# xyyandhtl/IsaacgymLoco

Hardware: AMD Instinct MI355X
Metric: env-steps/sec (whole node) (higher is better)
Workload: dtype f32; 1 GPU; aliengo: HIMOnPolicyRunner loop, 9 whole PPO iteration(s) timed, each = 100 x (policy inference + LeggedRobot.step + storage) + GAE + HIMPPO.update (5 epochs x 4 minibatches), 4096 envs/GPU; task=aliengo, envs_per_gpu=4096, mode=train, parallelism=dp1, mixed_robots=False, full=False

## Files before the change

### include/lsim.h

```cpp
#ifndef LSIM_H
#define LSIM_H

#include <stddef.h>
#include <stdint.h>

#ifdef __cplusplus
extern "C" {
#endif

#define LSIM_ABI_VERSION 7

#define LSIM_NUM_DOF 12
#define LSIM_NUM_BODIES 17
#define LSIM_NUM_LEGS 4
#define LSIM_NUM_ACTIONS 12
#define LSIM_ONE_STEP_OBS 45
#define LSIM_OBS_HISTORY 6
#define LSIM_NUM_OBS 270
#define LSIM_MAX_HEIGHT_PTS_X 32
#define LSIM_MAX_HEIGHT_PTS_Y 32
#define LSIM_NUM_HEIGHT_PTS 187
#define LSIM_NUM_PRIV_OBS 238
#define LSIM_NUM_AMP_OBS 30
#define LSIM_NUM_BASE_HEIGHT_PTS 63
// ... 473 lines not shown


int lsim_adaptive_lr(const float* kl_mean_dev, float desired_kl, float lr_min, float lr_max, float factor, float* lr_dev, void* stream);

int lsim_sinkhorn_workspace(long batch, int K, size_t* bytes);
int lsim_sinkhorn(const float* scores, int64_t lds, int64_t batch, int K, float eps, int iters, float* out,
                  void* workspace, size_t workspace_bytes, void* stream);

int lsim_estimator_loss_workspace(int64_t batch, int latent, int K, size_t* bytes);
int lsim_estimator_loss(const float* enc_out, int64_t ld_enc, const float* tgt_out, int64_t ld_tgt, const float* proto, const float* vel,
                        int64_t ld_vel, int64_t batch, int latent, int K, float temperature, float sinkhorn_eps, int sinkhorn_iters,
                        float* losses3, float* grad_enc, float* grad_tgt, float* grad_proto, void* workspace, size_t workspace_bytes,
                        void* stream);

int lsim_adam_clip_step_workspace(int count, size_t* bytes);
int lsim_adam_clip_step(int count, const int64_t* numel, float* const* params, float* const* grads, float* const* exp_avg,
                        float* const* exp_avg_sq, float* const* steps, const float* lr_dev, float lr_host, float beta1, float beta2,
                        float eps, float max_grad_norm, float* grad_norm_out, void* workspace, size_t workspace_bytes, void* stream);

int lsim_adam_clip_step_ex(int count, const int64_t* numel, float* const* params, float* const* grads, float* const* exp_avg,
                           float* const* exp_avg_sq, float* const* steps, const float* weight_decay, int clip_count,
                           const float* lr_dev, float lr_host, float beta1, float beta2, float eps, float max_grad_norm,
                           float* grad_norm_out, void* workspace, size_t workspace_bytes, void* stream);

int lsim_actor_input(const float* obs, int64_t ld_obs, int num_one_step_obs, const float* enc_out, int64_t ld_enc, int latent,
                     int64_t batch, float* out, void* stream);

#define LSIM_EVAL_BY_ROBOT 1u
#define LSIM_EVAL_BY_TYPE 2u
#define LSIM_EVAL_BY_LEVEL 4u
#define LSIM_EVAL_MAX_GROUPS 4096
#define LSIM_EVAL_MAX_TRACE_ENVS 64
#define LSIM_EVAL_SAT_PERMILLE 980
enum lsim_eval_word {
    LSIM_EVAL_W_SAMPLES = 0,
    LSIM_EVAL_W_LIN_ERR,
    LSIM_EVAL_W_LIN_ERR_SQ,
    LSIM_EVAL_W_YAW_ERR,
    LSIM_EVAL_W_YAW_ERR_SQ,
    LSIM_EVAL_W_POWER,
    LSIM_EVAL_W_TORQUE_SQ,
    LSIM_EVAL_W_ACTION_RATE,
    LSIM_EVAL_W_FEET_CONTACT,
    LSIM_EVAL_W_TORQUE_SAT,
    LSIM_EVAL_W_PEAK_TORQUE_RATIO,
    LSIM_EVAL_W_EPISODES,
// ... 516 lines not shown
```

### isaacgymloco_amd/abi.py

```python
import ctypes
import os
import re

_HERE = os.path.dirname(os.path.abspath(__file__))
REPO_ROOT = os.path.dirname(_HERE)
HEADER_PATH = os.path.join(REPO_ROOT, "include", "lsim.h")

_CTYPES = {
    "float": ctypes.c_float, "double": ctypes.c_double,
    "int32_t": ctypes.c_int32, "uint32_t": ctypes.c_uint32,
    "int64_t": ctypes.c_int64, "uint64_t": ctypes.c_uint64,
    "int16_t": ctypes.c_int16, "uint8_t": ctypes.c_uint8, "int": ctypes.c_int,
}


def _strip_comments(text):
    text = re.sub(r"/\*.*?\*/", "", text, flags=re.S)
    return re.sub(r"//[^\n]*", "", text)


def _parse(text, overrides=None):
    text = _strip_comments(text)
    defines = {}
    for m in re.finditer(r"^\s*#define\s+(\w+)\s+(.+?)\s*$", text, flags=re.M):
# ... 48 lines not shown
                decl = decl.strip()
                dm = re.match(r"(\w+)((?:\[[^\]]+\])*)$", decl)
                name, dims = dm.group(1), re.findall(r"\[([^\]]+)\]", dm.group(2))
                ct = base
                for d in reversed(dims):
                    ct = ct * int(eval(d, {}, defines))
                fields.append((name, ct))
        structs[m.group(3)] = type(m.group(3), (ctypes.Structure,), {"_fields_": fields})
    return defines, enums, structs


with open(HEADER_PATH) as _f:
    DEFINES, ENUMS, STRUCTS = _parse(_f.read())

LsimConfig = STRUCTS["lsim_config"]
LsimRobotModel = STRUCTS["lsim_robot_model"]
LsimBody = STRUCTS["lsim_body"]
LsimCollisionPoint = STRUCTS["lsim_collision_point"]
LsimRolloutStorage = STRUCTS["lsim_rollout_storage"]
LsimMlpLayer = STRUCTS["lsim_mlp_layer"]
LsimHimPolicy = STRUCTS["lsim_him_policy"]
LsimPolicyExtra = STRUCTS["lsim_policy_extra"]
LsimWgradPending = STRUCTS["lsim_wgrad_pending"]
LsimAmpDisc = STRUCTS["lsim_amp_disc"]
LsimEval = STRUCTS["lsim_eval"]
LsimEvalColumns = STRUCTS["lsim_eval_columns"]
LsimRaycast = STRUCTS["lsim_raycast_t"]
LsimRaycastBodies = STRUCTS["lsim_raycast_bodies_t"]
LsimRaycastRobot = STRUCTS["lsim_raycast_robot"]
LsimRaycastPrim = STRUCTS["lsim_raycast_prim"]
LsimSensorModel = STRUCTS["lsim_sensor_model_t"]
LsimSensorMountJitter = STRUCTS["lsim_sensor_mount_jitter_t"]
LsimSensorInstrument = STRUCTS["lsim_sensor_instrument_t"]
LsimSensorStereo = STRUCTS["lsim_sensor_stereo_t"]
LsimSensorShade = STRUCTS["lsim_sensor_shade_t"]
LsimElevationMap = STRUCTS["lsim_elevation_map_t"]
LsimOdometry = STRUCTS["lsim_odometry_t"]
LsimMapRows = STRUCTS["lsim_map_rows_t"]
LsimElevationMapFused = STRUCTS["lsim_elevation_map_fused_t"]
LsimMapRowsFused = STRUCTS["lsim_map_rows_fused_t"]
LsimElevationMapCleanup = STRUCTS["lsim_elevation_map_cleanup_t"]
LsimFootScan = STRUCTS["lsim_foot_scan_t"]
LsimDepthEncoder = STRUCTS["lsim_depth_encoder_t"]
LsimDepthEncoderBwd = STRUCTS["lsim_depth_encoder_bwd_t"]
LsimFramesLog = STRUCTS["lsim_frames_log_t"]
LsimLatentRowsGrad = STRUCTS["lsim_latent_rows_grad_t"]
# ... 89 lines not shown
```

### isaacgymloco_amd/csrc/ls_learn.h

```cpp
#pragma once
#include <hip/hip_runtime.h>

typedef float ls_v4f __attribute__((ext_vector_type(4)));

#define LS_WGRAD_WAVES_PER_BLOCK 4

template <int NT, int KT>
__global__ __launch_bounds__(64 * LS_WGRAD_WAVES_PER_BLOCK) void lsim_k_linear_wgrad(const float* __restrict__ x, long ldx, const float* __restrict__ g, long ldg,
                                                                                    long batch, int k_in, int n_out, long rows_per_wave,
                                                                                    float* __restrict__ part_dw, float* __restrict__ part_db) {
    const int lane = threadIdx.x & 63, wave = blockIdx.x * LS_WGRAD_WAVES_PER_BLOCK + (threadIdx.x >> 6);
    const int sub = lane >> 4, col = lane & 15;
    const long b0 = (long)wave * rows_per_wave;
    if (b0 >= batch) return;
    long b1 = b0 + rows_per_wave;
    if (b1 > batch) b1 = batch;
    ls_v4f acc[NT][KT];
    float dbacc[NT];
#pragma unroll
    for (int nt = 0; nt < NT; ++nt) {
        dbacc[nt] = 0.0f;
#pragma unroll
        for (int kt = 0; kt < KT; ++kt) acc[nt][kt] = (ls_v4f){0.0f, 0.0f, 0.0f, 0.0f};
    }
// ... 1428 lines not shown
    *bytes = (size_t)((batch + 255) / 256) * (4 + num_actions) * sizeof(float);
    return LSIM_OK;
}
extern "C" int lsim_ppo_loss_std(const float* mu, const float* std, const float* value, const float* actions, const float* old_logp, const float* advantages,
                                 const float* returns, const float* target_values, const float* old_mu, const float* old_sigma, int64_t batch, int num_actions,
                                 float clip_param, float value_loss_coef, float entropy_coef, int use_clipped_value_loss,
                                 float* out5, float* grad_mu, float* grad_std, float* grad_value, void* workspace, size_t workspace_bytes, void* stream) {
    size_t need;
    if (lsim_ppo_loss_std_workspace(batch, num_actions, &need) != LSIM_OK) return LSIM_E_INVALID;
    if (!mu || !std || !value || !actions || !old_logp || !advantages || !returns || !old_mu || !old_sigma || !out5 || !grad_mu || !grad_std ||
        !grad_value || !workspace || workspace_bytes < need || (use_clipped_value_loss && !target_values)) return LSIM_E_INVALID;
    LsPpoLossArgs a;
    a.mu = mu; a.sigma = std; a.value = value; a.actions = actions; a.old_logp = old_logp; a.adv = advantages; a.returns = returns;
    a.target_values = target_values; a.old_mu = old_mu; a.old_sigma = old_sigma; a.g_mu = grad_mu; a.g_sigma = nullptr; a.g_value = grad_value;
    a.partial = (float*)workspace; a.batch = batch; a.A = num_actions; a.clip = clip_param; a.value_coef = value_loss_coef;
    a.entropy_coef = entropy_coef; a.clipped_value = use_clipped_value_loss; a.std_mode = 1;
    const int blocks = (int)((batch + 255) / 256);
    hipLaunchKernelGGL(lsim_k_ppo_loss, dim3(blocks), dim3(256), 0, (hipStream_t)stream, a);
    hipLaunchKernelGGL(lsim_k_ppo_loss_finish_std, dim3(1), dim3(256), 0, (hipStream_t)stream, (const float*)workspace, blocks, (long)batch, num_actions,
                       value_loss_coef, entropy_coef, out5, grad_std);
    return hipGetLastError() == hipSuccess ? LSIM_OK : LSIM_E_HIP;
}

__global__ void lsim_k_adaptive_lr(const float* __restrict__ kl_mean, float desired_kl, float lr_min, float lr_max, float factor, float* __restrict__ lr) {
    const float k = *kl_mean;
    float l = *lr;
    if (k > 2.0f * desired_kl) l = fmaxf(lr_min, l / factor);
    else if (k < 0.5f * desired_kl && k > 0.0f) l = fminf(lr_max, l * factor);
    *lr = l;
}

extern "C" int lsim_adaptive_lr(const float* kl_mean_dev, float desired_kl, float lr_min, float lr_max, float factor, float* lr_dev, void* stream) {
    if (!kl_mean_dev || !lr_dev || desired_kl <= 0.0f || factor <= 1.0f || lr_min <= 0.0f || lr_max < lr_min) return LSIM_E_INVALID;
    hipLaunchKernelGGL(lsim_k_adaptive_lr, dim3(1), dim3(1), 0, (hipStream_t)stream, kl_mean_dev, desired_kl, lr_min, lr_max, factor, lr_dev);
    return hipGetLastError() == hipSuccess ? LSIM_OK : LSIM_E_HIP;
}

#define LS_ADAM_MAX_TENSORS 48
#define LS_ADAM_SLICES 32
struct LsAdamTable {
    float* p[LS_ADAM_MAX_TENSORS];
    float* g[LS_ADAM_MAX_TENSORS];
    float* m[LS_ADAM_MAX_TENSORS];
    float* v[LS_ADAM_MAX_TENSORS];
    float* step[LS_ADAM_MAX_TENSORS];
    int n[LS_ADAM_MAX_TENSORS];
    float wd[LS_ADAM_MAX_TENSORS];
    int count;
    int clip_count;
};

__global__ __launch_bounds__(256) void lsim_k_adam_sumsq(LsAdamTable t, float* __restrict__ part ) {
    __shared__ float red[256];
    const int ti = blockIdx.y, n = t.n[ti];
    const float* __restrict__ g = t.g[ti];
    float s = 0.0f;
    for (int i = blockIdx.x * 256 + threadIdx.x; i < n; i += LS_ADAM_SLICES * 256) { const float x = g[i]; s = fmaf(x, x, s); }
    red[threadIdx.x] = s;
    __syncthreads();
    for (int st = 128; st > 0; st >>= 1) {
        if ((int)threadIdx.x < st) red[threadIdx.x] += red[threadIdx.x + st];
        __syncthreads();
    }
    if (threadIdx.x == 0) {
        part[ti * LS_ADAM_SLICES + blockIdx.x] = red[0];
        if (blockIdx.x == 0) *t.step[ti] += 1.0f;
    }
}

__global__ __launch_bounds__(256) void lsim_k_adam_apply(LsAdamTable t, const float* __restrict__ part, float max_norm, float* __restrict__ scal,
                                                         const float* __restrict__ lr_dev, float lr_host, float b1, float b2, float eps) {
    __shared__ float tot[LS_ADAM_MAX_TENSORS];
    __shared__ float coef_s;
    if ((int)threadIdx.x < t.count) {
        float s = 0.0f;
        for (int k = 0; k < LS_ADAM_SLICES; ++k) s += part[threadIdx.x * LS_ADAM_SLICES + k];
        tot[threadIdx.x] = s;
    }
    __syncthreads();
    if (threadIdx.x == 0) {
        float s = 0.0f;
        for (int k = 0; k < t.clip_count; ++k) s += tot[k];
        const float norm = sqrtf(s);
        coef_s = max_norm > 0.0f ? fminf(max_norm / (norm + 1e-6f), 1.0f) : 1.0f;
        if (blockIdx.x == 0 && blockIdx.y == 0) { scal[0] = coef_s; scal[1] = norm; scal[2] = *t.step[0]; }
    }
    __syncthreads();
    const int ti = blockIdx.y, n = t.n[ti];
    float* __restrict__ p = t.p[ti];
    float* __restrict__ g = t.g[ti];
    float* __restrict__ m = t.m[ti];
    float* __restrict__ v = t.v[ti];
    const float coef = ti < t.clip_count ? coef_s : 1.0f, step = *t.step[ti], lr = lr_dev ? *lr_dev : lr_host, wd = t.wd[ti];
    const float bc1 = 1.0f - powf(b1, step), bc2s = sqrtf(1.0f - powf(b2, step));
    const float step_size = lr / bc1;
    for (int i = blockIdx.x * 256 + threadIdx.x; i < n; i += LS_ADAM_SLICES * 256) {
        const float gc = g[i] * coef;
        const float gi = wd != 0.0f ? gc + wd * p[i] : gc;
        const float mi = m[i] + (gi - m[i]) * (1.0f - b1);
        const float vi = b2 * v[i] + (1.0f - b2) * gi * gi;
        g[i] = gc; m[i] = mi; v[i] = vi;
        p[i] -= step_size * mi / (sqrtf(vi) / bc2s + eps);
    }
}

extern "C" int lsim_adam_clip_step_workspace(int count, size_t* bytes) {
    if (!bytes || count <= 0 || count > LS_ADAM_MAX_TENSORS) return LSIM_E_INVALID;
    *bytes = ((size_t)count * LS_ADAM_SLICES + 4) * sizeof(float);
    return LSIM_OK;
}

extern "C" int lsim_adam_clip_step_ex(int count, const int64_t* numel, float* const* params, float* const* grads, float* const* exp_avg,
                                      float* const* exp_avg_sq, float* const* steps, const float* weight_decay, int clip_count,
                                      const float* lr_dev, float lr_host, float beta1, float beta2, float eps, float max_grad_norm,
                                      float* grad_norm_out, void* workspace, size_t workspace_bytes, void* stream);
extern "C" int lsim_adam_clip_step(int count, const int64_t* numel, float* const* params, float* const* grads, float* const* exp_avg,
                                   float* const* exp_avg_sq, float* const* steps, const float* lr_dev, float lr_host, float beta1, float beta2,
                                   float eps, float max_grad_norm, float* grad_norm_out, void* workspace, size_t workspace_bytes, void* stream) {
    return lsim_adam_clip_step_ex(count, numel, params, grads, exp_avg, exp_avg_sq, steps, nullptr, count, lr_dev, lr_host, beta1, beta2, eps,
                                  max_grad_norm, grad_norm_out, workspace, workspace_bytes, stream);
}

extern "C" int lsim_adam_clip_step_ex(int count, const int64_t* numel, float* const* params, float* const* grads, float* const* exp_avg,
                                      float* const* exp_avg_sq, float* const* steps, const float* weight_decay, int clip_count,
                                      const float* lr_dev, float lr_host, float beta1, float beta2, float eps, float max_grad_norm,
                                      float* grad_norm_out, void* workspace, size_t workspace_bytes, void* stream) {
    size_t need;
    int rc = lsim_adam_clip_step_workspace(count, &need);
    if (rc != LSIM_OK) return rc;
    if (!numel || !params || !grads || !exp_avg || !exp_avg_sq || !steps || !workspace || workspace_bytes < need || beta1 < 0.0f || beta1 >= 1.0f ||
        beta2 < 0.0f || beta2 >= 1.0f || eps <= 0.0f || clip_count < 0 || clip_count > count)
        return LSIM_E_INVALID;
    LsAdamTable t;
    t.count = count;
    t.clip_count = clip_count;
    for (int i = 0; i < count; ++i) {
        if (!params[i] || !grads[i] || !exp_avg[i] || !exp_avg_sq[i] || !steps[i] || numel[i] <= 0 || numel[i] > 0x7fffffffLL) return LSIM_E_INVALID;
        t.p[i] = params[i]; t.g[i] = grads[i]; t.m[i] = exp_avg[i]; t.v[i] = exp_avg_sq[i]; t.step[i] = steps[i]; t.n[i] = (int)numel[i];
        t.wd[i] = weight_decay ? weight_decay[i] : 0.0f;
        if (t.wd[i] < 0.0f) return LSIM_E_INVALID;
    }
    for (int i = count; i < LS_ADAM_MAX_TENSORS; ++i) { t.p[i] = t.g[i] = t.m[i] = t.v[i] = t.step[i] = nullptr; t.n[i] = 0; t.wd[i] = 0.0f; }
    float* part = (float*)workspace;
    float* scal = part + (size_t)count * LS_ADAM_SLICES;
    hipStream_t s = (hipStream_t)stream;
    hipLaunchKernelGGL(lsim_k_adam_sumsq, dim3(LS_ADAM_SLICES, count), dim3(256), 0, s, t, part);
    hipLaunchKernelGGL(lsim_k_adam_apply, dim3(LS_ADAM_SLICES, count), dim3(256), 0, s, t, (const float*)part, max_grad_norm, scal, lr_dev, lr_host, beta1,
                       beta2, eps);
    if (grad_norm_out && hipMemcpyAsync(grad_norm_out, scal + 1, sizeof(float), hipMemcpyDeviceToDevice, s) != hipSuccess) return LSIM_E_HIP;
    return hipGetLastError() == hipSuccess ? LSIM_OK : LSIM_E_HIP;
}

__global__ __launch_bounds__(256) void lsim_k_actor_input(const float* __restrict__ obs, long ld_obs, int n_one, const float* __restrict__ enc, long ld_enc,
                                                          int n_lat, long batch, float* __restrict__ out) {
    const int W = n_one + 3 + n_lat;
    const long idx = (long)blockIdx.x * 256 + threadIdx.x;
    if (idx >= batch * W) return;
    const long row = idx / W;
    const int c = (int)(idx - row * W);
    float v;
    if (c < n_one) v = obs[row * ld_obs + c];
    else if (c < n_one + 3) v = enc[row * ld_enc + (c - n_one)];
    else {
        const float* z = enc + row * ld_enc + 3;
        float ss = 0.0f;
        for (int k = 0; k < n_lat; ++k) ss = fmaf(z[k], z[k], ss);
        v = z[c - n_one - 3] / fmaxf(sqrtf(ss), 1e-12f);
    }
    out[idx] = v;
}

__global__ __launch_bounds__(256) void lsim_k_actor_input64(const float* __restrict__ obs, long ld_obs, int n_one, const float* __restrict__ enc, long ld_enc,
// ... 27 lines not shown
```

### isaacgymloco_amd/learn/fused_linear.py

```python
import ctypes
import os
import weakref

import torch
import torch.nn as nn
import torch.nn.functional as F

_MIN_BATCH = 4096
_workspaces = {}
_plans = {}
_adam_tables = {}


def _workspace(kind, device, nbytes, floor=0):
    key = (kind, device, torch.cuda.current_stream(device).cuda_stream)
    ws = _workspaces.get(key)
    if ws is None or ws.numel() < nbytes:
        ws = torch.empty(max(int(nbytes), int(floor)), dtype=torch.uint8, device=device)
        _workspaces[key] = ws
    return ws


class GradArena:

# ... 373 lines not shown
    _EstimatorLossFn.last_grads = None
    return total, parts


def backward_losses(*losses):
    tensors, grads, rest = [], [], []
    direct = os.environ.get("LSIM_DIRECT_LOSS_BACKWARD", "1") != "0"
    for l in losses:
        d = getattr(l, "_lsim_direct", None) if direct else None
        if d is None or not all(t.requires_grad for t in d[0]):
            rest.append(l)
        else:
            tensors += list(d[0]); grads += list(d[1])
    if tensors:
        torch.autograd.backward(tensors, grads)
    for l in rest:
        l.backward()


def estimator_loss_supported(latent, K):
    return latent <= 32 and K <= 64


def adam_clip_step_hip(optimizer, max_grad_norm, clip_params=None):
    from .. import lib
    groups = optimizer.param_groups
    g0 = groups[0]
    for grp in groups:
        if grp.get("amsgrad") or grp.get("maximize") or grp.get("differentiable") or grp.get("weight_decay", 0) < 0:
            return False
        same_lr = grp["lr"] is g0["lr"] or (not torch.is_tensor(grp["lr"]) and not torch.is_tensor(g0["lr"]) and grp["lr"] == g0["lr"])
        if grp["betas"] != g0["betas"] or grp["eps"] != g0["eps"] or not same_lr:
            return False
    clip_ids = None if clip_params is None else {id(p) for p in clip_params}
    entries = [(p, float(grp.get("weight_decay", 0))) for grp in groups for p in grp["params"] if p.grad is not None]
    if not entries or len(entries) > 48:
        return False
    if clip_ids is not None:
        entries = [e for e in entries if id(e[0]) in clip_ids] + [e for e in entries if id(e[0]) not in clip_ids]
    n_clip = len(entries) if clip_ids is None else sum(1 for e in entries if id(e[0]) in clip_ids)
    n = len(entries)
    L = lib.load()
    dev = entries[0][0].device
    states = [optimizer.state.get(p) for p, _ in entries]
    for (p, _), st in zip(entries, states):
        if (not st or not p.is_cuda or p.dtype != torch.float32 or not p.is_contiguous() or not p.grad.is_contiguous()
                or not torch.is_tensor(st.get("step")) or not st["step"].is_cuda or st["step"].dtype != torch.float32):
            return False
    key = (n_clip, tuple(p.data_ptr() for p, _ in entries), tuple(p.grad.data_ptr() for p, _ in entries),
           tuple(st["exp_avg"].data_ptr() for st in states), tuple(st["exp_avg_sq"].data_ptr() for st in states),
           tuple(st["step"].data_ptr() for st in states), tuple(w for _, w in entries))
    cached = _adam_tables.get(id(optimizer))
    if cached is not None and cached[0] == key and cached[2]() is optimizer:
        tables = cached[1]
    else:
        tabs = ([], [], [], [], [])
        for (p, _), st in zip(entries, states):
            for tab, t in zip(tabs, (p, p.grad, st["exp_avg"], st["exp_avg_sq"], st["step"])):
                tab.append(t.data_ptr())
        need = ctypes.c_size_t()
        lib.check(L.lsim_adam_clip_step_workspace(n, ctypes.byref(need)), what="lsim_adam_clip_step_workspace")
        arr = lambda v: (ctypes.c_void_p * n)(*v)
        tables = (arr(tabs[0]), arr(tabs[1]), arr(tabs[2]), arr(tabs[3]), arr(tabs[4]), (ctypes.c_int64 * n)(*[p.numel() for p, _ in entries]),
                  (ctypes.c_float * n)(*[w for _, w in entries]), need.value)
        oid = id(optimizer)
        _adam_tables[oid] = (key, tables, weakref.ref(optimizer, lambda _r, oid=oid: _adam_tables.pop(oid, None)))
    ws = _workspace(("adam", id(optimizer)), dev, tables[7])
    lr = g0["lr"]
    lr_dev = lr.data_ptr() if torch.is_tensor(lr) and lr.is_cuda else None
    lr_host = 0.0 if lr_dev is not None else float(lr)
    b1, b2 = g0["betas"]
    lib.check(L.lsim_adam_clip_step_ex(n, tables[5], tables[0], tables[1], tables[2], tables[3], tables[4], tables[6], n_clip, lr_dev, lr_host,
                                       float(b1), float(b2), float(g0["eps"]), float(max_grad_norm), None, ws.data_ptr(), ws.numel(),
                                       torch.cuda.current_stream(dev).cuda_stream), what="lsim_adam_clip_step_ex")
    return True
```

### isaacgymloco_amd/learn/him_ppo.py

```python
import os
import time

import torch
import torch.nn as nn

from . import fused_linear as FL
from .storage import HIMRolloutStorage


_two_stream_memo = {}


def _loaded_tunableop_solutions(device):
    tun = torch.cuda.tunable
    a = torch.zeros(8, 8, device=device)
    torch.mm(a, a)
    table = {}
    for rec in tun.get_results():
        if len(rec) >= 3 and str(rec[0]).startswith("Gemm"):
            table[str(rec[1]).split("_ld_")[0]] = str(rec[2])
    return table


def tunableop_status(device, table_path=None):
# ... 171 lines not shown
        self.collectives += 1
        self.dist.all_reduce(v, op=self.dist.ReduceOp.SUM)
        v = v.to(torch.float32)
        return v[0], v[1], v[2]

    def sum_triple_vec(self, a, b, c):
        if not self.enabled:
            return a, b, c
        v = torch.cat((a.reshape(-1), b.reshape(-1), c.reshape(1))).to(torch.float64)
        self.collectives += 1
        self.dist.all_reduce(v, op=self.dist.ReduceOp.SUM)
        n = a.numel()
        return v[:n].view_as(a), v[n:2 * n].view_as(b), v[2 * n]

    def broadcast_module(self, module):
        if not self.enabled:
            return
        for t in list(module.parameters()) + list(module.buffers()):
            self.dist.broadcast(t.data, src=0)


class _Minibatch:
    __slots__ = ("obs", "next_critic_obs", "old_mu", "old_sigma", "loss", "mu", "sigma", "kl_mean", "surrogate_loss", "value_loss", "early_est", "aux",
                 "est", "swap", "est_params", "ppo_params", "kl", "dist", "bucket")

    def step_joint(self, alg, ac, more_params=()):
        alg._mb_backward(ac, self, more_params)
        alg._mb_reduce(self)
        alg._mb_optim(ac, self)


class HIMPPO:
    def __init__(self, actor_critic, num_learning_epochs=1, num_mini_batches=1, clip_param=0.2, gamma=0.998, lam=0.95,
                 value_loss_coef=1.0, entropy_coef=0.0, learning_rate=1e-3, max_grad_norm=1.0, use_clipped_value_loss=True,
                 schedule="fixed", desired_kl=0.01, device="cpu", dist_ctx=None):
        self.device = device
        self.desired_kl, self.schedule, self.learning_rate = desired_kl, schedule, learning_rate
        self.actor_critic = actor_critic.to(device)
        self.storage = None
        self.optimizer = torch.optim.Adam(self.actor_critic.parameters(), lr=learning_rate)
        self.transition = HIMRolloutStorage.Transition()
        self.clip_param, self.num_learning_epochs, self.num_mini_batches = clip_param, num_learning_epochs, num_mini_batches
        self.value_loss_coef, self.entropy_coef, self.gamma, self.lam = value_loss_coef, entropy_coef, gamma, lam
        self.max_grad_norm, self.use_clipped_value_loss = max_grad_norm, use_clipped_value_loss
        self.dist_ctx = dist_ctx
        self._lr_t = None
        if dist_ctx is not None and dist_ctx.enabled:
# ... 171 lines not shown
        est_ids = {id(p) for p in est_params}
        ppo_params = [p for p in ac.parameters() if p.grad is not None and id(p) not in est_ids]
        more = [p for p in more_params if p.grad is not None]
        mb.est, mb.swap, mb.est_params, mb.ppo_params, mb.kl, mb.bucket = est.detach(), swap.detach(), est_params, ppo_params, extra, None
        mb.dist = (mb.mu, mb.sigma, mb.old_mu, mb.old_sigma) if self._lr_t is None else (None,) * 4
        if ctx is not None:
            slot = self._stats_slot()
            in_place = slot is not None and extra is not None and extra.data_ptr() == slot[3:4].data_ptr()
            mb.bucket = ctx.prepare_bucket(est_live + ppo_params + more, extra=None if in_place else extra, key="all",
                                           n_extra=5 if (extra is not None and extra.is_cuda) else None, extra_at=3)
        elif self._grad_arena() is not None:
            self._arena.bucket("all", est_live + ppo_params + more, 0).adopt()

    def _mb_reduce(self, mb):
        if mb.bucket is None:
            return
        ctx = self.dist_ctx
        got = ctx.finish_bucket(ctx.start_reduce(mb.bucket))
        if mb.kl is not None:
            mb.kl = got[3:4] if got.numel() == 5 else got

    def _mb_optim(self, ac, mb):
        est_mod = ac.estimator
        if self._adaptive:
            self._adapt_lr(*mb.dist, mb.kl.reshape(()), already_global=True)
        if self._lr_t is None:
            est_mod.learning_rate = self.learning_rate
            for g in est_mod.optimizer.param_groups:
                g["lr"] = self.learning_rate
        stepped = False
        if est_mod.fused_step:
            stepped = FL.adam_clip_step_hip(est_mod.optimizer, est_mod.max_grad_norm)
        if not stepped:
            nn.utils.clip_grad_norm_(mb.est_params, est_mod.max_grad_norm)
            est_mod.optimizer.step()
        for p in mb.est_params:
            p.grad = None
        self._clip_and_step(self.optimizer, mb.ppo_params, self.max_grad_norm)

    def _mb_step_single_rank(self, ac, mb, bucket_params, clip_params):
        if self._adaptive:
            self._adapt_lr(mb.mu, mb.sigma, mb.old_mu, mb.old_sigma, mb.kl_mean)
        mb.est, mb.swap = ac.estimator.update(mb.obs, mb.next_critic_obs, lr=None if self._lr_t is not None else self.learning_rate)
        self._extra_losses(mb)
        self.optimizer.zero_grad()
        FL.grad_cycle()
        with FL.deferred_wgrad_reduce():
            FL.backward_losses(mb.loss)
        if FL._arena is not None:
            FL._arena.bucket("ppo", [p for p in bucket_params if p.grad is not None]).adopt()
        self._clip_and_step(self.optimizer, clip_params, self.max_grad_norm)

    _std_direct = True
    _two_stream_forward = True

    def _mb_forward(self, ac, batch, two_streams):
        (obs, critic_obs, actions, next_critic_obs, target_values, advantages, returns, old_logp, old_mu, old_sigma) = batch
        if two_streams:
            cur = torch.cuda.current_stream(obs.device)
            side = self._side_stream(obs.device)
            side.wait_stream(cur)
# ... 24 lines not shown
    _n_stats = 4

    def _sample_stream(self):
        for batch in self.storage.mini_batch_generator(self.num_mini_batches, self.num_learning_epochs):
            yield batch, None

    def _extra_losses(self, mb):
        return ()

    def _after_step(self, ac, mb):
        """behind the optimiser steps of a minibatch"""

    def _stats_row(self, mb):
        return mb.value_loss.detach(), mb.surrogate_loss.detach(), mb.est, mb.swap

    def _result(self, means, mb):
        return means[0], means[1], float(mb.est), float(mb.swap)

    def update(self):
        ac = self.actor_critic
        t_enqueue = time.perf_counter()
        self._grad_arena()
        sums = torch.zeros(self._n_stats, device=self.device)
        dist_on = self.dist_ctx is not None and self.dist_ctx.enabled
        for batch, aux in self._sample_stream():
            obs = batch[0]
            two_streams = (self._two_stream_forward and obs.is_cuda and self._lr_t is not None
                           and self._two_streams(ac.critic, obs.shape[0], dist_on and self.dist_ctx.world > 1))
            mb = self._mb_forward(ac, batch, two_streams)
            mb.aux = aux
            if dist_on or two_streams:
                mb.step_joint(self, ac, self._extra_losses(mb))
            else:
                self._mb_step_single_rank(ac, mb, [p for g in self.optimizer.param_groups for p in g["params"]], ac.parameters())
            self._after_step(ac, mb)
            sums += torch.stack(self._stats_row(mb))
        n = self.num_learning_epochs * self.num_mini_batches
        self.update_enqueue_s = time.perf_counter() - t_enqueue
        if self._lr_t is not None:
            self.learning_rate = float(self._lr_t)
        means = (sums / n).tolist()
        self.storage.clear()
        return self._result(means, mb)
```

### isaacgymloco_amd/learn/hybrid.py

```python
import torch
import torch.nn as nn

from .amp import AMPDiscriminator, AMPLoader, Normalizer, ReplayBuffer, default_motion_files
from .him_ppo import HIMPPO
from .modules import HIMActorCritic
from .runner import HIMOnPolicyRunner
from .storage import HIMRolloutStorage


class HybridPPO(HIMPPO):
    def __init__(self, actor_critic, discriminator, amp_data, amp_normalizer, amp_replay_buffer_size=100000, min_std=None,
                 device="cpu", dist_ctx=None, **kw):
        super().__init__(actor_critic, device=device, dist_ctx=dist_ctx, **kw)
        self.min_std = min_std
        self.discriminator = discriminator.to(device)
        self.amp_transition = HIMRolloutStorage.Transition()
        self.amp_storage = ReplayBuffer(discriminator.input_dim // 2, amp_replay_buffer_size, device)
        self.amp_data, self.amp_normalizer = amp_data, amp_normalizer
        self.optimizer = torch.optim.Adam([
            {"params": self.actor_critic.parameters(), "name": "actor_critic"},
            {"params": self.discriminator.trunk.parameters(), "weight_decay": 10e-4, "name": "amp_trunk"},
            {"params": self.discriminator.amp_linear.parameters(), "weight_decay": 10e-2, "name": "amp_head"}], lr=self.learning_rate)
        if dist_ctx is not None and dist_ctx.enabled:
            dist_ctx.broadcast_module(self.discriminator)
            if amp_normalizer is not None:
                amp_normalizer.moment_sync = lambda a, b, c: tuple(t.to(torch.float64) for t in dist_ctx.sum_triple_vec(a, b, c))

    def act(self, obs, critic_obs, amp_obs):
        self.amp_transition.observations = amp_obs
        return super().act(obs, critic_obs)

    def process_env_step(self, rewards, dones, infos, amp_obs, next_critic_obs):
        self.amp_storage.insert(self.amp_transition.observations, amp_obs)
        self.amp_transition.clear()
        super().process_env_step(rewards, dones, infos, next_critic_obs)

    _std_direct = False
    _two_stream_forward = False
    _n_stats = 6

    def _sample_stream(self):
        n_updates, rows = self.num_learning_epochs * self.num_mini_batches, self.storage.num_envs * self.storage.num_transitions_per_env // self.num_mini_batches
        for sample, policy_pair, expert_pair in zip(self.storage.mini_batch_generator(self.num_mini_batches, self.num_learning_epochs),
                                                    self.amp_storage.feed_forward_generator(n_updates, rows),
                                                    self.amp_data.feed_forward_generator(n_updates, rows)):
            yield sample, (policy_pair, expert_pair)

    def _extra_losses(self, mb):
        disc = self.discriminator
        (pol_s, pol_ns), (exp_s_raw, exp_ns_raw) = mb.aux
        expert_in, policy_in, expert_raw, exp_s, pol_s = disc.pair_inputs(exp_s_raw, exp_ns_raw, pol_s, pol_ns, self.amp_normalizer)
        amp_loss, policy_d_mean, expert_d_mean = disc.lsgan_loss(expert_in, policy_in)
        grad_pen = disc.compute_grad_pen(exp_s_raw, exp_ns_raw, lambda_=10, pair=expert_raw)
        mb.loss = mb.loss + amp_loss + grad_pen
        mb.aux = (pol_s, exp_s, amp_loss.detach(), grad_pen.detach(), policy_d_mean, expert_d_mean)
        return disc.parameters()

    def _after_step(self, ac, mb):
        if self.min_std is not None:
            ac.std.data = ac.std.data.clamp(min=self.min_std)
        if self.amp_normalizer is not None:
# ... 91 lines not shown
```

Before: 4.945 million env-steps/s.

## Fuse adaptive LR, two Adam clip steps and stat accumulation into one tail

Adds a combined update-tail entry point that runs the estimator and PPO Adam clip-steps as two kernels covering both optimizers together. The first kernel also applies the adaptive learning-rate rule and accumulates the per-minibatch loss statistics. The HIM PPO minibatch optimizer path calls it when possible, which removes several small kernel launches and torch.stack/add ops per minibatch. The Adam element loop is unrolled by four. Risks are tighter eligibility checks that can fall back to the old path, and a small reordering in the arithmetic because fp contraction is now explicit.

```diff
diff --git a/include/lsim.h b/include/lsim.h
--- a/include/lsim.h
+++ b/include/lsim.h
@@ -519,6 +519,22 @@
                            float* const* exp_avg_sq, float* const* steps, const float* weight_decay, int clip_count,
                            const float* lr_dev, float lr_host, float beta1, float beta2, float eps, float max_grad_norm,
                            float* grad_norm_out, void* workspace, size_t workspace_bytes, void* stream);
+
+typedef struct lsim_adam_group {
+    int32_t count, clip_count;
+    const int64_t* numel;
+    float** params;
+    float** grads;
+    float** exp_avg;
+    float** exp_avg_sq;
+    float** steps;
+    const float* weight_decay;
+    float beta1, beta2, eps, max_grad_norm;
+} lsim_adam_group;
+int lsim_update_tail_workspace(int count0, int count1, size_t* bytes);
+int lsim_update_tail(const lsim_adam_group* groups, int num_groups, float* lr_dev, const float* kl_mean_dev, float desired_kl, float lr_min,
+                     float lr_max, float factor, const float* const* stat_src, float* stat_sums, void* workspace, size_t workspace_bytes,
+                     void* stream);
 
 int lsim_actor_input(const float* obs, int64_t ld_obs, int num_one_step_obs, const float* enc_out, int64_t ld_enc, int latent,
                      int64_t batch, float* out, void* stream);
diff --git a/isaacgymloco_amd/abi.py b/isaacgymloco_amd/abi.py
--- a/isaacgymloco_amd/abi.py
+++ b/isaacgymloco_amd/abi.py
@@ -94,6 +94,7 @@
 LsimHimPolicy = STRUCTS["lsim_him_policy"]
 LsimPolicyExtra = STRUCTS["lsim_policy_extra"]
 LsimWgradPending = STRUCTS["lsim_wgrad_pending"]
+LsimAdamGroup = STRUCTS["lsim_adam_group"]
 LsimAmpDisc = STRUCTS["lsim_amp_disc"]
 LsimEval = STRUCTS["lsim_eval"]
 LsimEvalColumns = STRUCTS["lsim_eval_columns"]
diff --git a/isaacgymloco_amd/csrc/ls_learn.h b/isaacgymloco_amd/csrc/ls_learn.h
--- a/isaacgymloco_amd/csrc/ls_learn.h
+++ b/isaacgymloco_amd/csrc/ls_learn.h
@@ -1474,12 +1474,14 @@
     return hipGetLastError() == hipSuccess ? LSIM_OK : LSIM_E_HIP;
 }
 
-__global__ void lsim_k_adaptive_lr(const float* __restrict__ kl_mean, float desired_kl, float lr_min, float lr_max, float factor, float* __restrict__ lr) {
-    const float k = *kl_mean;
-    float l = *lr;
+__device__ __forceinline__ float ls_adaptive_lr(float k, float l, float desired_kl, float lr_min, float lr_max, float factor) {
     if (k > 2.0f * desired_kl) l = fmaxf(lr_min, l / factor);
     else if (k < 0.5f * desired_kl && k > 0.0f) l = fminf(lr_max, l * factor);
-    *lr = l;
+    return l;
+}
+
+__global__ void lsim_k_adaptive_lr(const float* __restrict__ kl_mean, float desired_kl, float lr_min, float lr_max, float factor, float* __restrict__ lr) {
+    *lr = ls_adaptive_lr(*kl_mean, *lr, desired_kl, lr_min, lr_max, factor);
 }
 
 extern "C" int lsim_adaptive_lr(const float* kl_mean_dev, float desired_kl, float lr_min, float lr_max, float factor, float* lr_dev, void* stream) {
@@ -1502,10 +1504,7 @@
     int clip_count;
 };
 
-__global__ __launch_bounds__(256) void lsim_k_adam_sumsq(LsAdamTable t, float* __restrict__ part ) {
-    __shared__ float red[256];
-    const int ti = blockIdx.y, n = t.n[ti];
-    const float* __restrict__ g = t.g[ti];
+__device__ __forceinline__ float ls_adam_sumsq_slice(const float* __restrict__ g, int n, float* red ) {
     float s = 0.0f;
     for (int i = blockIdx.x * 256 + threadIdx.x; i < n; i += LS_ADAM_SLICES * 256) { const float x = g[i]; s = fmaf(x, x, s); }
     red[threadIdx.x] = s;
@@ -1514,46 +1513,87 @@
         if ((int)threadIdx.x < st) red[threadIdx.x] += red[threadIdx.x + st];
         __syncthreads();
     }
+    return red[0];
+}
+
+__global__ __launch_bounds__(256) void lsim_k_adam_sumsq(LsAdamTable t, float* __restrict__ part ) {
+    __shared__ float red[256];
+    const int ti = blockIdx.y;
+    const float s = ls_adam_sumsq_slice(t.g[ti], t.n[ti], red);
     if (threadIdx.x == 0) {
-        part[ti * LS_ADAM_SLICES + blockIdx.x] = red[0];
+        part[ti * LS_ADAM_SLICES + blockIdx.x] = s;
         if (blockIdx.x == 0) *t.step[ti] += 1.0f;
     }
+}
+
+__device__ __forceinline__ float ls_adam_coef(const float* __restrict__ part, int count, int clip_count, float max_norm, float* tot ,
+                                              float* coef_s ) {
+    float norm = 0.0f;
+    if ((int)threadIdx.x < count) {
+        float s = 0.0f;
+        for (int k = 0; k < LS_ADAM_SLICES; ++k) s += part[threadIdx.x * LS_ADAM_SLICES + k];
+        tot[threadIdx.x] = s;
+    }
+    __syncthreads();
+    if (threadIdx.x == 0) {
+        float s = 0.0f;
+        for (int k = 0; k < clip_count; ++k) s += tot[k];
+        norm = sqrtf(s);
+        *coef_s = max_norm > 0.0f ? fminf(max_norm / (norm + 1e-6f), 1.0f) : 1.0f;
+    }
+    __syncthreads();
+    return norm;
+}
+
+struct LsAdamScalars { float coef, wd, b1, b2, eps, step_size, bc2s; };
+__device__ __forceinline__ LsAdamScalars ls_adam_scalars(float coef, float step, float lr, float wd, float b1, float b2, float eps) {
+    LsAdamScalars a;
+    const float bc1 = 1.0f - powf(b1, step);
+    a.coef = coef; a.wd = wd; a.b1 = b1; a.b2 = b2; a.eps = eps;
+    a.bc2s = sqrtf(1.0f - powf(b2, step));
+    a.step_size = lr / bc1;
+    return a;
+}
+
+__device__ __forceinline__ void ls_adam_element(const LsAdamScalars& a, float& g, float& m, float& v, float& p) {
+#pragma clang fp contract(off)
+    const float gc = g * a.coef;
+    const float gi = a.wd != 0.0f ? fmaf(a.wd, p, gc) : gc;
+    const float mi = fmaf(1.0f - a.b1, gi - m, m);
+    const float vi = fmaf(gi, (1.0f - a.b2) * gi, a.b2 * v);
+    g = gc; m = mi; v = vi;
+    p -= a.step_size * mi / (sqrtf(vi) / a.bc2s + a.eps);
 }
 
 __global__ __launch_bounds__(256) void lsim_k_adam_apply(LsAdamTable t, const float* __restrict__ part, float max_norm, float* __restrict__ scal,
                                                          const float* __restrict__ lr_dev, float lr_host, float b1, float b2, float eps) {
     __shared__ float tot[LS_ADAM_MAX_TENSORS];
     __shared__ float coef_s;
-    if ((int)threadIdx.x < t.count) {
-        float s = 0.0f;
-        for (int k = 0; k < LS_ADAM_SLICES; ++k) s += part[threadIdx.x * LS_ADAM_SLICES + k];
-        tot[threadIdx.x] = s;
-    }
-    __syncthreads();
-    if (threadIdx.x == 0) {
-        float s = 0.0f;
-        for (int k = 0; k < t.clip_count; ++k) s += tot[k];
-        const float norm = sqrtf(s);
-        coef_s = max_norm > 0.0f ? fminf(max_norm / (norm + 1e-6f), 1.0f) : 1.0f;
-        if (blockIdx.x == 0 && blockIdx.y == 0) { scal[0] = coef_s; scal[1] = norm; scal[2] = *t.step[0]; }
-    }
-    __syncthreads();
+    const float norm = ls_adam_coef(part, t.count, t.clip_count, max_norm, tot, &coef_s);
+    if (threadIdx.x == 0 && blockIdx.x == 0 && blockIdx.y == 0) { scal[0] = coef_s; scal[1] = norm; scal[2] = *t.step[0]; }
     const int ti = blockIdx.y, n = t.n[ti];
     float* __restrict__ p = t.p[ti];
     float* __restrict__ g = t.g[ti];
     float* __restrict__ m = t.m[ti];
     float* __restrict__ v = t.v[ti];
-    const float coef = ti < t.clip_count ? coef_s : 1.0f, step = *t.step[ti], lr = lr_dev ? *lr_dev : lr_host, wd = t.wd[ti];
-    const float bc1 = 1.0f - powf(b1, step), bc2s = sqrtf(1.0f - powf(b2, step));
-    const float step_size = lr / bc1;
+    const LsAdamScalars a = ls_adam_scalars(ti < t.clip_count ? coef_s : 1.0f, *t.step[ti], lr_dev ? *lr_dev : lr_host, t.wd[ti], b1, b2, eps);
     for (int i = blockIdx.x * 256 + threadIdx.x; i < n; i += LS_ADAM_SLICES * 256) {
-        const float gc = g[i] * coef;
-        const float gi = wd != 0.0f ? gc + wd * p[i] : gc;
-        const float mi = m[i] + (gi - m[i]) * (1.0f - b1);
-        const float vi = b2 * v[i] + (1.0f - b2) * gi * gi;
-        g[i] = gc; m[i] = mi; v[i] = vi;
-        p[i] -= step_size * mi / (sqrtf(vi) / bc2s + eps);
-    }
+        float gi = g[i], mi = m[i], vi = v[i], pi = p[i];
+        ls_adam_element(a, gi, mi, vi, pi);
+        g[i] = gi; m[i] = mi; v[i] = vi; p[i] = pi;
+    }
+}
+
+static bool ls_adam_group_ok(int count, const int64_t* numel, float* const* params, float* const* grads, float* const* exp_avg, float* const* exp_avg_sq,
+                             float* const* steps, const float* weight_decay, int clip_count, float beta1, float beta2, float eps) {
+    if (!numel || !params || !grads || !exp_avg || !exp_avg_sq || !steps || beta1 < 0.0f || beta1 >= 1.0f || beta2 < 0.0f || beta2 >= 1.0f ||
+        eps <= 0.0f || clip_count < 0 || clip_count > count)
+        return false;
+    for (int i = 0; i < count; ++i)
+        if (!params[i] || !grads[i] || !exp_avg[i] || !exp_avg_sq[i] || !steps[i] || numel[i] <= 0 || numel[i] > 0x7fffffffLL ||
+            (weight_decay && weight_decay[i] < 0.0f))
+            return false;
+    return true;
 }
 
 extern "C" int lsim_adam_clip_step_workspace(int count, size_t* bytes) {
@@ -1580,17 +1620,15 @@
     size_t need;
     int rc = lsim_adam_clip_step_workspace(count, &need);
     if (rc != LSIM_OK) return rc;
-    if (!numel || !params || !grads || !exp_avg || !exp_avg_sq || !steps || !workspace || workspace_bytes < need || beta1 < 0.0f || beta1 >= 1.0f ||
-        beta2 < 0.0f || beta2 >= 1.0f || eps <= 0.0f || clip_count < 0 || clip_count > count)
+    if (!workspace || workspace_bytes < need || !ls_adam_group_ok(count, numel, params, grads, exp_avg, exp_avg_sq, steps, weight_decay, clip_count,
+                                                                  beta1, beta2, eps))
         return LSIM_E_INVALID;
     LsAdamTable t;
     t.count = count;
     t.clip_count = clip_count;
     for (int i = 0; i < count; ++i) {
-        if (!params[i] || !grads[i] || !exp_avg[i] || !exp_avg_sq[i] || !steps[i] || numel[i] <= 0 || numel[i] > 0x7fffffffLL) return LSIM_E_INVALID;
         t.p[i] = params[i]; t.g[i] = grads[i]; t.m[i] = exp_avg[i]; t.v[i] = exp_avg_sq[i]; t.step[i] = steps[i]; t.n[i] = (int)numel[i];
         t.wd[i] = weight_decay ? weight_decay[i] : 0.0f;
-        if (t.wd[i] < 0.0f) return LSIM_E_INVALID;
     }
     for (int i = count; i < LS_ADAM_MAX_TENSORS; ++i) { t.p[i] = t.g[i] = t.m[i] = t.v[i] = t.step[i] = nullptr; t.n[i] = 0; t.wd[i] = 0.0f; }
     float* part = (float*)workspace;
@@ -1600,6 +1638,136 @@
     hipLaunchKernelGGL(lsim_k_adam_apply, dim3(LS_ADAM_SLICES, count), dim3(256), 0, s, t, (const float*)part, max_grad_norm, scal, lr_dev, lr_host, beta1,
                        beta2, eps);
     if (grad_norm_out && hipMemcpyAsync(grad_norm_out, scal + 1, sizeof(float), hipMemcpyDeviceToDevice, s) != hipSuccess) return LSIM_E_HIP;
+    return hipGetLastError() == hipSuccess ? LSIM_OK : LSIM_E_HIP;
+}
+
+#define LS_TAIL_MAX_TENSORS (2 * LS_ADAM_MAX_TENSORS)
+#define LS_TAIL_UNROLL 4
+struct LsTailSumsqTable {
+    const float* g[LS_TAIL_MAX_TENSORS];
+    float* step[LS_TAIL_MAX_TENSORS];
+    int n[LS_TAIL_MAX_TENSORS];
+};
+struct LsTailApplyTable {
+    float* p[LS_TAIL_MAX_TENSORS];
+    float* g[LS_TAIL_MAX_TENSORS];
+    float* m[LS_TAIL_MAX_TENSORS];
+    float* v[LS_TAIL_MAX_TENSORS];
+    int n[LS_TAIL_MAX_TENSORS];
+    float wd[LS_TAIL_MAX_TENSORS];
+};
+struct LsTailGroup { int count, clip_count; float max_norm, b1, b2, eps; };
+struct LsTailScalars {
+    const float* kl; float* lr; float desired_kl, lr_min, lr_max, factor;
+    const float* src[4]; float* sums;
+};
+__host__ __device__ inline size_t ls_tail_group_floats(int count) { return count > 0 ? (size_t)count * LS_ADAM_SLICES + 4 : 0; }
+
+__global__ __launch_bounds__(256) void lsim_k_tail_sumsq(LsTailSumsqTable t, LsTailScalars sc, int count0, int count1, float* __restrict__ ws) {
+    __shared__ float red[256];
+    const int ti = blockIdx.y;
+    const float s = ls_adam_sumsq_slice(t.g[ti], t.n[ti], red);
+    if (threadIdx.x != 0) return;
+    float* part = ti < count0 ? ws + (size_t)ti * LS_ADAM_SLICES : ws + ls_tail_group_floats(count0) + (size_t)(ti - count0) * LS_ADAM_SLICES;
+    part[blockIdx.x] = s;
+    if (blockIdx.x != 0) return;
+    const float st = *t.step[ti] + 1.0f;
+    *t.step[ti] = st;
+    (ws + ls_tail_group_floats(count0) + ls_tail_group_floats(count1))[ti] = st;
+    if (ti != 0) return;
+    if (sc.kl) *sc.lr = ls_adaptive_lr(*sc.kl, *sc.lr, sc.desired_kl, sc.lr_min, sc.lr_max, sc.factor);
+    if (sc.sums)
+        for (int k = 0; k < 4; ++k) sc.sums[k] += *sc.src[k];
+}
+
+__global__ __launch_bounds__(256) void lsim_k_tail_apply(LsTailApplyTable t, LsTailGroup g0, LsTailGroup g1, const float* __restrict__ lr,
+                                                         float* __restrict__ ws) {
+    __shared__ float tot[LS_ADAM_MAX_TENSORS];
+    __shared__ float coef_s;
+    const int ti = blockIdx.y;
+    const bool second = ti >= g0.count;
+    const LsTailGroup G = second ? g1 : g0;
+    const int local = second ? ti - g0.count : ti;
+    float* part = second ? ws + ls_tail_group_floats(g0.count) : ws;
+    const float* stepv = ws + ls_tail_group_floats(g0.count) + ls_tail_group_floats(g1.count);
+    const float norm = ls_adam_coef(part, G.count, G.clip_count, G.max_norm, tot, &coef_s);
+    if (threadIdx.x == 0 && blockIdx.x == 0 && local == 0) {
+        float* scal = part + (size_t)G.count * LS_ADAM_SLICES;
+        scal[0] = coef_s; scal[1] = norm; scal[2] = stepv[ti];
+    }
+    const long n = t.n[ti], stride = LS_ADAM_SLICES * 256;
+    float* p = t.p[ti];
+    float* g = t.g[ti];
+    float* m = t.m[ti];
+    float* v = t.v[ti];
+    const LsAdamScalars a = ls_adam_scalars(local < G.clip_count ? coef_s : 1.0f, stepv[ti], *lr, t.wd[ti], G.b1, G.b2, G.eps);
+    for (long i0 = blockIdx.x * 256 + threadIdx.x; i0 < n; i0 += LS_TAIL_UNROLL * stride) {
+        float gi[LS_TAIL_UNROLL], mi[LS_TAIL_UNROLL], vi[LS_TAIL_UNROLL], pi[LS_TAIL_UNROLL];
+#pragma unroll
+        for (int u = 0; u < LS_TAIL_UNROLL; ++u) {
+            const long i = i0 + u * stride;
+            if (i < n) { gi[u] = g[i]; mi[u] = m[i]; vi[u] = v[i]; pi[u] = p[i]; }
+        }
+#pragma unroll
+        for (int u = 0; u < LS_TAIL_UNROLL; ++u) {
+            const long i = i0 + u * stride;
+            if (i < n) {
+                ls_adam_element(a, gi[u], mi[u], vi[u], pi[u]);
+                g[i] = gi[u]; m[i] = mi[u]; v[i] = vi[u]; p[i] = pi[u];
+            }
+        }
+    }
+}
+
+extern "C" int lsim_update_tail_workspace(int count0, int count1, size_t* bytes) {
+    if (!bytes || count0 <= 0 || count0 > LS_ADAM_MAX_TENSORS || count1 < 0 || count1 > LS_ADAM_MAX_TENSORS) return LSIM_E_INVALID;
+    *bytes = (ls_tail_group_floats(count0) + ls_tail_group_floats(count1) + (size_t)(count0 + count1)) * sizeof(float);
+    return LSIM_OK;
+}
+
+extern "C" int lsim_update_tail(const lsim_adam_group* groups, int num_groups, float* lr_dev, const float* kl_mean_dev, float desired_kl, float lr_min,
+                                float lr_max, float factor, const float* const* stat_src, float* stat_sums, void* workspace, size_t workspace_bytes,
+                                void* stream) {
+    const auto aligned = [](const void* q) { return ((uintptr_t)q & 3u) == 0; };
+    if (!groups || num_groups < 1 || num_groups > 2 || !lr_dev || !aligned(lr_dev) || !workspace || !aligned(workspace)) return LSIM_E_INVALID;
+    if (kl_mean_dev && (!aligned(kl_mean_dev) || desired_kl <= 0.0f || factor <= 1.0f || lr_min <= 0.0f || lr_max < lr_min)) return LSIM_E_INVALID;
+    if ((stat_src != nullptr) != (stat_sums != nullptr) || !aligned(stat_sums)) return LSIM_E_INVALID;
+    size_t need;
+    if (lsim_update_tail_workspace(groups[0].count, num_groups == 2 ? groups[1].count : 0, &need) != LSIM_OK || (num_groups == 2 && groups[1].count <= 0) ||
+        workspace_bytes < need)
+        return LSIM_E_INVALID;
+    LsTailSumsqTable ts;
+    LsTailApplyTable ta;
+    LsTailGroup tg[2] = {};
+    LsTailScalars sc = {};
+    int total = 0;
+    for (int k = 0; k < num_groups; ++k) {
+        const lsim_adam_group& G = groups[k];
+        if (!ls_adam_group_ok(G.count, G.numel, G.params, G.grads, G.exp_avg, G.exp_avg_sq, G.steps, G.weight_decay, G.clip_count, G.beta1, G.beta2, G.eps))
+            return LSIM_E_INVALID;
+        tg[k].count = G.count; tg[k].clip_count = G.clip_count; tg[k].max_norm = G.max_grad_norm; tg[k].b1 = G.beta1; tg[k].b2 = G.beta2; tg[k].eps = G.eps;
+        for (int i = 0; i < G.count; ++i, ++total) {
+            if (!aligned(G.params[i]) || !aligned(G.grads[i]) || !aligned(G.exp_avg[i]) || !aligned(G.exp_avg_sq[i]) || !aligned(G.steps[i])) return LSIM_E_INVALID;
+            ts.g[total] = ta.g[total] = G.grads[i]; ts.step[total] = G.steps[i]; ts.n[total] = ta.n[total] = (int)G.numel[i];
+            ta.p[total] = G.params[i]; ta.m[total] = G.exp_avg[i]; ta.v[total] = G.exp_avg_sq[i]; ta.wd[total] = G.weight_decay ? G.weight_decay[i] : 0.0f;
+        }
+    }
+    for (int i = total; i < LS_TAIL_MAX_TENSORS; ++i) {
+        ts.g[i] = nullptr; ts.step[i] = nullptr; ts.n[i] = ta.n[i] = 0;
+        ta.p[i] = ta.g[i] = ta.m[i] = ta.v[i] = nullptr; ta.wd[i] = 0.0f;
+    }
+    sc.lr = lr_dev;
+    if (kl_mean_dev) { sc.kl = kl_mean_dev; sc.desired_kl = desired_kl; sc.lr_min = lr_min; sc.lr_max = lr_max; sc.factor = factor; }
+    if (stat_src) {
+        for (int k = 0; k < 4; ++k) {
+            if (!stat_src[k] || !aligned(stat_src[k])) return LSIM_E_INVALID;
+            sc.src[k] = stat_src[k];
+        }
+        sc.sums = stat_sums;
+    }
+    hipStream_t s = (hipStream_t)stream;
+    hipLaunchKernelGGL(lsim_k_tail_sumsq, dim3(LS_ADAM_SLICES, total), dim3(256), 0, s, ts, sc, tg[0].count, tg[1].count, (float*)workspace);
+    hipLaunchKernelGGL(lsim_k_tail_apply, dim3(LS_ADAM_SLICES, total), dim3(256), 0, s, ta, tg[0], tg[1], (const float*)lr_dev, (float*)workspace);
     return hipGetLastError() == hipSuccess ? LSIM_OK : LSIM_E_HIP;
 }
 
diff --git a/isaacgymloco_amd/learn/fused_linear.py b/isaacgymloco_amd/learn/fused_linear.py
--- a/isaacgymloco_amd/learn/fused_linear.py
+++ b/isaacgymloco_amd/learn/fused_linear.py
@@ -419,20 +419,20 @@
     return latent <= 32 and K <= 64
 
 
-def adam_clip_step_hip(optimizer, max_grad_norm, clip_params=None):
+def _adam_call(optimizer, clip_params=None, skip_ids=()):
     from .. import lib
     groups = optimizer.param_groups
     g0 = groups[0]
     for grp in groups:
         if grp.get("amsgrad") or grp.get("maximize") or grp.get("differentiable") or grp.get("weight_decay", 0) < 0:
-            return False
+            return None
         same_lr = grp["lr"] is g0["lr"] or (not torch.is_tensor(grp["lr"]) and not torch.is_tensor(g0["lr"]) and grp["lr"] == g0["lr"])
         if grp["betas"] != g0["betas"] or grp["eps"] != g0["eps"] or not same_lr:
-            return False
+            return None
     clip_ids = None if clip_params is None else {id(p) for p in clip_params}
-    entries = [(p, float(grp.get("weight_decay", 0))) for grp in groups for p in grp["params"] if p.grad is not None]
+    entries = [(p, float(grp.get("weight_decay", 0))) for grp in groups for p in grp["params"] if p.grad is not None and id(p) not in skip_ids]
     if not entries or len(entries) > 48:
-        return False
+        return None
     if clip_ids is not None:
         entries = [e for e in entries if id(e[0]) in clip_ids] + [e for e in entries if id(e[0]) not in clip_ids]
     n_clip = len(entries) if clip_ids is None else sum(1 for e in entries if id(e[0]) in clip_ids)
@@ -443,7 +443,7 @@
     for (p, _), st in zip(entries, states):
         if (not st or not p.is_cuda or p.dtype != torch.float32 or not p.is_contiguous() or not p.grad.is_contiguous()
                 or not torch.is_tensor(st.get("step")) or not st["step"].is_cuda or st["step"].dtype != torch.float32):
-            return False
+            return None
     key = (n_clip, tuple(p.data_ptr() for p, _ in entries), tuple(p.grad.data_ptr() for p, _ in entries),
            tuple(st["exp_avg"].data_ptr() for st in states), tuple(st["exp_avg_sq"].data_ptr() for st in states),
            tuple(st["step"].data_ptr() for st in states), tuple(w for _, w in entries))
@@ -462,6 +462,16 @@
                   (ctypes.c_float * n)(*[w for _, w in entries]), need.value)
         oid = id(optimizer)
         _adam_tables[oid] = (key, tables, weakref.ref(optimizer, lambda _r, oid=oid: _adam_tables.pop(oid, None)))
+    return tables, n, n_clip, g0, dev
+
+
+def adam_clip_step_hip(optimizer, max_grad_norm, clip_params=None):
+    from .. import lib
+    call = _adam_call(optimizer, clip_params)
+    if call is None:
+        return False
+    tables, n, n_clip, g0, dev = call
+    L = lib.load()
     ws = _workspace(("adam", id(optimizer)), dev, tables[7])
     lr = g0["lr"]
     lr_dev = lr.data_ptr() if torch.is_tensor(lr) and lr.is_cuda else None
@@ -471,3 +481,43 @@
                                        float(b1), float(b2), float(g0["eps"]), float(max_grad_norm), None, ws.data_ptr(), ws.numel(),
                                        torch.cuda.current_stream(dev).cuda_stream), what="lsim_adam_clip_step_ex")
     return True
+
+
+_tail_groups = {}
+
+
+def update_tail_hip(first, second, lr_t, kl=None, lr_rule=None, stats=None, sums=None):
+    from .. import abi, lib
+    scalar = lambda t, n=1: torch.is_tensor(t) and t.is_cuda and t.dtype == torch.float32 and t.numel() == n and t.is_contiguous()
+    if not scalar(lr_t) or (kl is not None and not scalar(kl)) or (stats is not None and not (len(stats) == 4 and all(scalar(t) for t in stats)
+                                                                                               and scalar(sums, 4))):
+        return False
+    calls = []
+    for opt, _, clip_params, skip_ids in (first, second):
+        calls.append(_adam_call(opt, clip_params, skip_ids))
+        if calls[-1] is None or calls[-1][3]["lr"] is not lr_t:
+            return False
+    L = lib.load()
+    key = tuple((id(c[0]), c[1], c[2], float(o[1]), tuple(c[3]["betas"]), float(c[3]["eps"])) for c, o in zip(calls, (first, second)))
+    oid = (id(first[0]), id(second[0]))
+    cached = _tail_groups.get(oid)
+    if cached is not None and cached[0] == key and cached[2]() is first[0] and cached[3]() is second[0]:
+        groups, need = cached[1]
+    else:
+        groups = (abi.LsimAdamGroup * 2)()
+        for G, (tables, n, n_clip, g0, _), o in zip(groups, calls, (first, second)):
+            G.count, G.clip_count = n, n_clip
+            G.numel, G.params, G.grads, G.exp_avg, G.exp_avg_sq, G.steps, G.weight_decay = (ctypes.addressof(tables[i]) for i in (5, 0, 1, 2, 3, 4, 6))
+            G.beta1, G.beta2, G.eps, G.max_grad_norm = float(g0["betas"][0]), float(g0["betas"][1]), float(g0["eps"]), float(o[1])
+        need = ctypes.c_size_t()
+        lib.check(L.lsim_update_tail_workspace(calls[0][1], calls[1][1], ctypes.byref(need)), what="lsim_update_tail_workspace")
+        need = need.value
+        drop = lambda _r, oid=oid: _tail_groups.pop(oid, None)
+        _tail_groups[oid] = (key, (groups, need), weakref.ref(first[0], drop), weakref.ref(second[0], drop), [c[0] for c in calls])
+    dev = calls[0][4]
+    ws = _workspace(("update_tail",) + oid, dev, need)
+    rule = (kl.data_ptr(),) + tuple(float(x) for x in lr_rule) if kl is not None else (None, 0.0, 0.0, 0.0, 0.0)
+    src = (ctypes.c_void_p * 4)(*[t.data_ptr() for t in stats]) if stats is not None else None
+    lib.check(L.lsim_update_tail(groups, 2, lr_t.data_ptr(), *rule, src, sums.data_ptr() if stats is not None else None, ws.data_ptr(), ws.numel(),
+                                 torch.cuda.current_stream(dev).cuda_stream), what="lsim_update_tail")
+    return True
diff --git a/isaacgymloco_amd/learn/him_ppo.py b/isaacgymloco_amd/learn/him_ppo.py
--- a/isaacgymloco_amd/learn/him_ppo.py
+++ b/isaacgymloco_amd/learn/him_ppo.py
@@ -217,7 +217,7 @@
 
 class _Minibatch:
     __slots__ = ("obs", "next_critic_obs", "old_mu", "old_sigma", "loss", "mu", "sigma", "kl_mean", "surrogate_loss", "value_loss", "early_est", "aux",
-                 "est", "swap", "est_params", "ppo_params", "kl", "dist", "bucket")
+                 "est", "swap", "est_params", "ppo_params", "kl", "dist", "bucket", "folded")
 
     def step_joint(self, alg, ac, more_params=()):
         alg._mb_backward(ac, self, more_params)
@@ -435,6 +435,8 @@
 
     def _mb_optim(self, ac, mb):
         est_mod = ac.estimator
+        if self._update_tail(est_mod, mb):
+            return
         if self._adaptive:
             self._adapt_lr(*mb.dist, mb.kl.reshape(()), already_global=True)
         if self._lr_t is None:
@@ -450,6 +452,22 @@
         for p in mb.est_params:
             p.grad = None
         self._clip_and_step(self.optimizer, mb.ppo_params, self.max_grad_norm)
+
+    _fused_tail = True
+
+    def _update_tail(self, est_mod, mb):
+        if not self._fused_tail or self._lr_t is None or not est_mod.fused_step or (self._adaptive and mb.kl is None):
+            return False
+        sums = getattr(self, "_stat_sums", None)
+        if not FL.update_tail_hip((est_mod.optimizer, est_mod.max_grad_norm, None, ()),
+                                  (self.optimizer, self.max_grad_norm, mb.ppo_params, {id(p) for p in mb.est_params}), self._lr_t,
+                                  kl=mb.kl.detach() if self._adaptive else None, lr_rule=(self.desired_kl, 1e-5, 1e-2, 1.5),
+                                  stats=self._stats_row(mb) if sums is not None else None, sums=sums):
+            return False
+        mb.folded = sums is not None
+        for p in mb.est_params:
+            p.grad = None
+        return True
 
     def _mb_step_single_rank(self, ac, mb, bucket_params, clip_params):
         if self._adaptive:
@@ -520,19 +538,22 @@
         t_enqueue = time.perf_counter()
         self._grad_arena()
         sums = torch.zeros(self._n_stats, device=self.device)
+        self._stat_sums = sums if self._n_stats == 4 else None
         dist_on = self.dist_ctx is not None and self.dist_ctx.enabled
         for batch, aux in self._sample_stream():
             obs = batch[0]
             two_streams = (self._two_stream_forward and obs.is_cuda and self._lr_t is not None
                            and self._two_streams(ac.critic, obs.shape[0], dist_on and self.dist_ctx.world > 1))
             mb = self._mb_forward(ac, batch, two_streams)
-            mb.aux = aux
+            mb.aux, mb.folded = aux, False
             if dist_on or two_streams:
                 mb.step_joint(self, ac, self._extra_losses(mb))
             else:
                 self._mb_step_single_rank(ac, mb, [p for g in self.optimizer.param_groups for p in g["params"]], ac.parameters())
             self._after_step(ac, mb)
-            sums += torch.stack(self._stats_row(mb))
+            if not mb.folded:
+                sums += torch.stack(self._stats_row(mb))
+        self._stat_sums = None
         n = self.num_learning_epochs * self.num_mini_batches
         self.update_enqueue_s = time.perf_counter() - t_enqueue
         if self._lr_t is not None:
diff --git a/isaacgymloco_amd/learn/hybrid.py b/isaacgymloco_amd/learn/hybrid.py
--- a/isaacgymloco_amd/learn/hybrid.py
+++ b/isaacgymloco_amd/learn/hybrid.py
@@ -37,6 +37,7 @@
 
     _std_direct = False
     _two_stream_forward = False
+    _fused_tail = False
     _n_stats = 6
 
     def _sample_stream(self):
```

New measurement: 4.937 million env-steps/s. No clear change (-0.2%).
